# DrorT/demucs

Hardware: AMD Instinct MI355X
Metric: real-time factor (audio-sec/wall-sec) htdemucs 4-stem 44.1kHz stereo, 1/8 GPU (higher is better)
Workload: dtype f32

## Files before the change

### demucs_amd/csrc/gemm_x6.hip

```cpp
#include "gemm_tile.h"
#include "split_bf16.h"

namespace mi {

typedef __attribute__((address_space(1))) const void gvoid_t;
typedef __attribute__((address_space(3))) void lvoid_t;

__global__ void pack_split_kernel(const float *__restrict__ wt, int Kpad, int Mpad, int BM, __bf16 *__restrict__ wx) {
    const size_t idx = blockIdx.x * (size_t)blockDim.x + threadIdx.x;
    if (idx >= (size_t)Kpad * Mpad) return;
    const int k = (int)(idx / Mpad), m = (int)(idx % Mpad);
    const int mt = m / BM, mi = m % BM, kt = k / BK, h = (k % BK) / 8, j = k % 8, nk = Kpad / BK;
    const float x = wt[idx];
    const __bf16 a = (__bf16)x;
    const float r = x - (float)a;
    const __bf16 b = (__bf16)r;
    const __bf16 c = (__bf16)(r - (float)b);
    __bf16 *img = wx + ((size_t)mt * nk + kt) * ((size_t)BM * 48);
    img[((0 * 2 + h) * BM + mi) * 8 + j] = a;
    img[((1 * 2 + h) * BM + mi) * 8 + j] = b;
    img[((2 * 2 + h) * BM + mi) * 8 + j] = c;
}

int launch_pack_split(const float *wt, int Kpad, int Mpad, int tile_m, void *wx, hipStream_t st) {
    MI_REQUIRE(Kpad % BK == 0 && Mpad % tile_m == 0, "pack_split: Kpad %d / Mpad %d do not fit tile %d", Kpad, Mpad, tile_m);
    const size_t n = (size_t)Kpad * Mpad;
    hipLaunchKernelGGL(pack_split_kernel, dim3((unsigned)((n + 255) / 256)), dim3(256), 0, st, wt, Kpad, Mpad, tile_m, (__bf16 *)wx);
    MI_CHECK_LAUNCH();
    return MI_OK;
}

#ifndef MI_X6_ABL
#define MI_X6_ABL 0
#endif
constexpr int kRowTaps = -1;
template <int WM, int WN, int TM, int TN, int EPI, int LFLAGS, bool PLAIN, bool HALF_IMG, int NT>
__device__ __forceinline__ void conv_x6_body(const mi_conv_desc &d, const int N, const int MT, const int Gm) {
    constexpr int BM = WM * TM * 32;
    constexpr bool RAW = PLAIN || NT != 0;
    constexpr bool ROWS = NT == kRowTaps;
    static_assert(NT <= 0 || (!PLAIN && EPI == MI_EPI_GLU), "tap loader: GLU rewrite convs");
    static_assert(!ROWS || (!PLAIN && (EPI == MI_EPI_LINEAR || EPI == MI_EPI_CONVTR || EPI == MI_EPI_GLU)),
                  "row-tap loader: encoder / transposed convs, 1 x 1 + GLU rewrites");
    static_assert(NT >= kRowTaps, "NT: taps, 0 or kRowTaps");
    static_assert(WN * TN * 32 == BN, "block N tile is 128");
    static_assert(WM * WN == 4, "4 waves");
    constexpr int A_BYTES = BM * 96, B_BYTES = BN * 96, STAGE = A_BYTES + B_BYTES;
    constexpr int A_CHUNKS = A_BYTES / 1024;
    static_assert(!HALF_IMG || BM == 64, "HALF_IMG: 64-row tile of a 128-row image");
    constexpr int A_KSTEP = HALF_IMG ? 2 * A_BYTES : A_BYTES, A_CHUNK_STRIDE = HALF_IMG ? 2048 : 1024;
    __shared__ __attribute__((aligned(16))) unsigned char smem[2 * STAGE];
    __shared__ __attribute__((aligned(16))) float braw[RAW ? 2 * BK * BN : 4];

    {
        float agpr_anchor = 0.f;
        asm volatile("; accumulators in AGPRs %0" : "+a"(agpr_anchor));
    }
    const int tid = threadIdx.x, lane = tid & 63;
    const int wave = __builtin_amdgcn_readfirstlane(tid >> 6);
    const int wm = wave / WN, wn = wave % WN;
    int mt, nt;
    if (!tile_of_block(MT, Gm, N, mt, nt)) return;
    const int m0 = mt * BM, n0 = nt * BN;
    const int P = d.O1 * d.O2;
    const int o2v = d.o2_valid ? d.o2_valid : d.O2;
    const int nk = d.Kpad / BK;

    const unsigned char *aimg = reinterpret_cast<const unsigned char *>(d.wx) + (size_t)(HALF_IMG ? mt >> 1 : mt) * nk * A_KSTEP +
                                (HALF_IMG ? (mt & 1) * 1024 : 0) + lane * 16;
#define MI_A_DMA(kt, stage)                                                                                         \
    do {                                                                                                            \
        _Pragma("unroll") for (int c = 0; c < (A_CHUNKS + 3) / 4; ++c) {                                             \
            const int chunk = c * 4 + wave;                                                                         \
            if (chunk < A_CHUNKS)                                                                                   \
                __builtin_amdgcn_global_load_lds((gvoid_t *)(aimg + (size_t)(kt) * A_KSTEP + chunk * A_CHUNK_STRIDE), \
                                                 (lvoid_t *)(smem + (stage) * STAGE + chunk * 1024), 16, 0, 0);     \
        }                                                                                                           \
    } while (0)

    const int bn = tid & 127;
    const int bh = __builtin_amdgcn_readfirstlane(tid >> 7);
    const ColInfo lc = decompose(n0 + bn, N, P, d.O2, PLAIN ? d.O2 : o2v);
    const int i1b = lc.o1 * d.S1, i2b = lc.o2 * d.S2;
    const float *xcol = d.x + (size_t)lc.b * d.x_bstride + (PLAIN ? (size_t)lc.p : (size_t)i1b * (d.x_ld ? d.x_ld : d.D2) + i2b);
    const float *bp = lc.valid ? xcol + (size_t)(8 * bh) * P : d.sink + 256;
    const size_t b_row = lc.valid ? (size_t)P : 0, b_step = lc.valid ? (size_t)BK * P : 0;
    float breg[8];
    const int li = lane & 31, lh = lane >> 5;
    const int rc4 = li * 4, rrow = 4 * wave + lh;
    const ColInfo rcol = decompose(n0 + rc4, N, P, d.O2, NT ? o2v : d.O2);
    const int x_ld = d.x_ld ? d.x_ld : d.D2;
    const int ri1 = rcol.o1 * d.S1;
    const float *rsrc = !rcol.valid ? d.sink + 256
                        : d.x + (size_t)rcol.b * d.x_bstride +
                              (ROWS ? (size_t)ri1 * x_ld + rcol.o2 : (size_t)rcol.p + (NT ? 0 : (size_t)rrow * P));
    const size_t r_row2 = rcol.valid ? (size_t)2 * P : 0, r_step = rcol.valid ? (size_t)BK * P : 0;
    const int4 *ktab4 = reinterpret_cast<const int4 *>(d.ktab) + 4 * wave;
    typedef int v2i __attribute__((ext_vector_type(2)));
    v2i e0, e1, e2, e3;
#define MI_ROW_LOADS "s_load_dwordx2 %0, %4, 0x0\n\ts_load_dwordx2 %1, %4, 0x10\n\ts_load_dwordx2 %2, %4, 0x20\n\t" \
                     "s_load_dwordx2 %3, %4, 0x30\n\t"
#define MI_ROW_ENTRIES(kt)                                                                                          \
    asm volatile(MI_ROW_LOADS "s_waitcnt lgkmcnt(0)"                                                               \
                 : "=&s"(e0), "=&s"(e1), "=&s"(e2), "=&s"(e3) : "s"(ktab4 + (kt) * BK) : "memory")
    constexpr int K2 = 3;
    const int fix_l = (NT && rcol.valid && rcol.o2 == 0) ? 0 : -1;
    const int fr = d.D2 - 1 - rcol.o2;
    const int fix_r = (NT && rcol.valid && fr >= 0 && fr < 4) ? fr : -1;
#define MI_BRAW_DMA(kt, rs)                                                                                         \
    do {                                                                                                            \
        float *dst = braw + (rs) * (BK * BN) + (4 * wave) * BN;                                                     \
        if constexpr (ROWS) {                                                                                       \
            _Pragma("unroll") for (int i = 0; i < 2; ++i) {                                                         \
                const int off = i ? (lh ? e3.x : e2.x) : (lh ? e1.x : e0.x);                                        \
                const int dd1 = i ? (lh ? e3.y : e2.y) : (lh ? e1.y : e0.y);                                        \
                const bool ok = rcol.valid && (unsigned)(ri1 + dd1) < (unsigned)d.D1;                               \
                __builtin_amdgcn_global_load_lds((gvoid_t *)(ok ? rsrc + off : d.sink + 256), (lvoid_t *)(dst + 2 * i * BN), 16, 0, 0); \
            }                                                                                                       \
        } else if constexpr (NT > 0) {                                                                              \
            _Pragma("unroll") for (int i = 0; i < 2; ++i) {                                                         \
                const int k = (kt) * BK + rrow + 2 * i, ci = k / NT, tap = k - ci * NT, t1 = tap / K2, t2 = tap - t1 * K2; \
                const int i1 = rcol.o1 + t1 - d.tap_pad1;                                                           \
                const bool ok = rcol.valid && k < d.K && (unsigned)i1 < (unsigned)d.D1;                             \
                const float *g = rsrc + (int64_t)ci * P + (int64_t)(t1 - d.tap_pad1) * x_ld + (t2 - d.tap_pad2);    \
                __builtin_amdgcn_global_load_lds((gvoid_t *)(ok ? g : d.sink + 256), (lvoid_t *)(dst + 2 * i * BN), 16, 0, 0); \
            }                                                                                                       \
        } else {                                                                                                    \
            const float *g = rsrc + (size_t)(kt) * r_step;                                                          \
            __builtin_amdgcn_global_load_lds((gvoid_t *)g, (lvoid_t *)dst, 16, 0, 0);                               \
            __builtin_amdgcn_global_load_lds((gvoid_t *)(g + r_row2), (lvoid_t *)(dst + 2 * BN), 16, 0, 0);         \
        }                                                                                                           \
    } while (0)
#define MI_BRAW_FIX(kt, rs)                                                                                         \
    do {                                                                                                            \
        if constexpr (NT > 0) {                                                                                     \
            float *row = braw + (rs) * (BK * BN) + rrow * BN + rc4;                                                 \
            _Pragma("unroll") for (int i = 0; i < 2; ++i) {                                                         \
                const int k = (kt) * BK + rrow + 2 * i, dd2 = (k % NT) % K2 - d.tap_pad2;                           \
                if (dd2 < 0 && fix_l >= 0) row[2 * i * BN + fix_l] = 0.f;                                           \
                if (dd2 > 0 && fix_r >= 0) row[2 * i * BN + fix_r] = 0.f;                                           \
            }                                                                                                       \
        }                                                                                                           \
    } while (0)
#define MI_BRAW_READ(rs)                                                                                            \
    do {                                                                                                            \
        _Pragma("unroll") for (int j = 0; j < 8; ++j) breg[j] = braw[(rs) * (BK * BN) + (8 * bh + j) * BN + bn];     \
    } while (0)

#define MI_B_LOAD(kt)                                                                                               \
    do {                                                                                                            \
        if (PLAIN) {                                                                                                \
            _Pragma("unroll") for (int j = 0; j < 8; ++j) breg[j] = bp[(size_t)(kt) * b_step + j * b_row];           \
        } else {                                                                                                    \
            mi_ktab_entry ke[8];                                                                                    \
            _Pragma("unroll") for (int j = 0; j < 8; ++j) ke[j] = d.ktab[(kt) * BK + 8 * bh + j];                    \
            _Pragma("unroll") for (int j = 0; j < 8; ++j) {                                                          \
                bool ok;                                                                                            \
                const float v = gather_b(d, ke[j], xcol, i1b, i2b, lc.valid, ok);                                   \
                breg[j] = ok ? v : 0.f;                                                                             \
            }                                                                                                       \
        }                                                                                                           \
    } while (0)

#define MI_B_STORE(stage)                                                                                           \
    do {                                                                                                            \
        unsigned ph[4], pm[4], pl[4];                                                                               \
        _Pragma("unroll") for (int j = 0; j < 4; ++j) split3(breg[2 * j], breg[2 * j + 1], ph[j], pm[j], pl[j]);    \
        unsigned char *bs = smem + (stage) * STAGE + A_BYTES + (bh * BN + bn) * 16;                                 \
        *reinterpret_cast<uint4 *>(bs) = make_uint4(ph[0], ph[1], ph[2], ph[3]);                                    \
        *reinterpret_cast<uint4 *>(bs + 2 * BN * 16) = make_uint4(pm[0], pm[1], pm[2], pm[3]);                      \
        *reinterpret_cast<uint4 *>(bs + 4 * BN * 16) = make_uint4(pl[0], pl[1], pl[2], pl[3]);                      \
    } while (0)

    f32x16 acc[TM][TN];
#pragma unroll
    for (int a = 0; a < TM; ++a)
#pragma unroll
        for (int b = 0; b < TN; ++b)
#pragma unroll
            for (int r = 0; r < 16; ++r) acc[a][b][r] = 0.f;

    constexpr int PA[6] = {2, 0, 1, 1, 0, 0}, PB[6] = {0, 2, 1, 0, 1, 0};
    MI_A_DMA(0, 0);
    if constexpr (RAW) {
        if constexpr (ROWS) MI_ROW_ENTRIES(0);
        MI_BRAW_DMA(0, 0);
        if (nk > 1) {
            if constexpr (ROWS) MI_ROW_ENTRIES(1);
            MI_BRAW_DMA(1, 1);
        }
        if constexpr (ROWS) { if (nk > 2) MI_ROW_ENTRIES(2); }
        asm volatile("s_waitcnt vmcnt(0)" ::: "memory");
        MI_BRAW_FIX(0, 0);
        if (nk > 1) MI_BRAW_FIX(1, 1);
        __syncthreads();
        MI_BRAW_READ(0);
    } else {
        MI_B_LOAD(0);
    }
    MI_B_STORE(0);
    asm volatile("s_waitcnt vmcnt(0)" ::: "memory");
    __syncthreads();
    int cur = 0;
    bf16x8 keepa[TM][3], keepb[TN][3];
    for (int kt = 0; kt < nk; ++kt) {
        const unsigned char *As = smem + cur * STAGE, *Bs = As + A_BYTES;
        bf16x8 af[TM][3], bf[TN][3];
        if ((MI_X6_ABL & 128) && kt > 0) {
#pragma unroll
            for (int p = 0; p < 3; ++p) {
#pragma unroll
                for (int a = 0; a < TM; ++a) af[a][p] = keepa[a][p];
#pragma unroll
                for (int b = 0; b < TN; ++b) bf[b][p] = keepb[b][p];
            }
        } else
#pragma unroll
        for (int p = 0; p < 3; ++p) {
#pragma unroll
            for (int a = 0; a < TM; ++a)
                af[a][p] = *reinterpret_cast<const bf16x8 *>(As + (((p * 2 + lh) * BM) + (wm * TM + a) * 32 + li) * 16);
#pragma unroll
            for (int b = 0; b < TN; ++b)
                bf[b][p] = *reinterpret_cast<const bf16x8 *>(Bs + (((p * 2 + lh) * BN) + (wn * TN + b) * 32 + li) * 16);
        }
        if (MI_X6_ABL & 128) {
#pragma unroll
            for (int p = 0; p < 3; ++p) {
#pragma unroll
                for (int a = 0; a < TM; ++a) keepa[a][p] = af[a][p];
#pragma unroll
                for (int b = 0; b < TN; ++b) keepb[b][p] = bf[b][p];
            }
        }
        if (MI_X6_ABL & 64) {
            typedef unsigned u32x4 __attribute__((ext_vector_type(4)));
#pragma unroll
            for (int p = 0; p < 3; ++p) {
#pragma unroll
                for (int a = 0; a < TM; ++a) { u32x4 z = __builtin_bit_cast(u32x4, af[a][p]); asm volatile("" : "+v"(z)); af[a][p] = __builtin_bit_cast(bf16x8, z); }
#pragma unroll
                for (int b = 0; b < TN; ++b) { u32x4 z = __builtin_bit_cast(u32x4, bf[b][p]); asm volatile("" : "+v"(z)); bf[b][p] = __builtin_bit_cast(bf16x8, z); }
            }
        }
        if (MI_X6_ABL & 8) {
            typedef unsigned u32x4 __attribute__((ext_vector_type(4)));
#pragma unroll
            for (int p = 0; p < 3; ++p) {
#pragma unroll
                for (int a = 0; a < TM; ++a) { u32x4 z = {0u, 0u, 0u, 0u}; asm volatile("" : "+v"(z)); af[a][p] = __builtin_bit_cast(bf16x8, z); }
#pragma unroll
                for (int b = 0; b < TN; ++b) { u32x4 z = {0u, 0u, 0u, 0u}; asm volatile("" : "+v"(z)); bf[b][p] = __builtin_bit_cast(bf16x8, z); }
            }
        }
        __builtin_amdgcn_sched_barrier(0);
        if (kt + 1 < nk) {
            MI_A_DMA(kt + 1, cur ^ 1);
            if constexpr (RAW) {
                if (kt + 2 < nk) MI_BRAW_DMA(kt + 2, kt & 1);
            } else {
                MI_B_LOAD(kt + 1);
            }
        }
        if constexpr (RAW) {
            MI_BRAW_READ((kt + 1) & 1);
        }
        __builtin_amdgcn_sched_barrier(0);
#pragma unroll
        for (int q = 0; q < 6; ++q)
#pragma unroll
            for (int a = 0; a < TM; ++a)
#pragma unroll
                for (int b = 0; b < TN; ++b)
                    if (!(MI_X6_ABL & 1) || (q == 0 && a == 0 && b == 0)) {
                        acc[a][b] = __builtin_amdgcn_mfma_f32_32x32x16_bf16(af[a][PA[q]], bf[b][PB[q]], acc[a][b], 0, 0, 0);
                        if (MI_X6_ABL & 16) asm volatile("s_nop 15\n\ts_nop 15");
                        if ((MI_X6_ABL & 32) && a == TM - 1 && b == TN - 1) asm volatile("s_nop 15\n\ts_nop 15\n\ts_nop 15\n\ts_nop 15");
                    }
        if (RAW || kt + 1 < nk) MI_B_STORE(cur ^ 1);
        if constexpr (RAW) {
#pragma unroll
            for (int i = 0; i < 6 * TM * TN; ++i) {
                __builtin_amdgcn_sched_group_barrier(0x008, 1, 0);
                __builtin_amdgcn_sched_group_barrier(0x002, (72 + 6 * TM * TN - 1) / (6 * TM * TN), 0);
            }
        }
        if (ROWS && kt + 3 < nk)
            asm volatile(MI_ROW_LOADS "s_waitcnt vmcnt(0) lgkmcnt(0)"
                         : "=&s"(e0), "=&s"(e1), "=&s"(e2), "=&s"(e3) : "s"(ktab4 + (kt + 3) * BK) : "memory");
        else
            asm volatile("s_waitcnt vmcnt(0)" ::: "memory");
        if (kt + 2 < nk) MI_BRAW_FIX(kt + 2, kt & 1);
        __syncthreads();
        cur ^= 1;
    }
#undef MI_A_DMA
#undef MI_B_LOAD
#undef MI_BRAW_DMA
#undef MI_BRAW_FIX
#undef MI_BRAW_READ
#undef MI_ROW_ENTRIES
#undef MI_ROW_LOADS
#undef MI_B_STORE

    if (MI_X6_ABL & 4) {
        float s = 0.f;
        for (int a = 0; a < TM; ++a) for (int b = 0; b < TN; ++b) for (int r = 0; r < 16; ++r) s += acc[a][b][r];
        d.sink[threadIdx.x] = s;
        return;
    }
    conv_epilogue<TM, TN, EPI, LFLAGS>(d, acc, m0, n0, wm, wn, N, P, o2v);
}

template <int WM, int WN, int TM, int TN, int EPI, int LFLAGS, bool PLAIN, bool HALF_IMG = false>
__global__ __launch_bounds__(256, 2) void conv_gemm_x6_kernel(const mi_conv_desc d, const int N, const int MT, const int Gm) {
    conv_x6_body<WM, WN, TM, TN, EPI, LFLAGS, PLAIN, HALF_IMG, 0>(d, N, MT, Gm);
}

template <int WM, int WN, int TM, int TN, bool HALF_IMG, int NT>
__global__ __launch_bounds__(256, 2) void conv_tap_x6_kernel(const mi_conv_desc d, const int N, const int MT, const int Gm) {
    conv_x6_body<WM, WN, TM, TN, MI_EPI_GLU, 0, false, HALF_IMG, NT>(d, N, MT, Gm);
}

template <int WM, int WN, int TM, int TN, int EPI, int LFLAGS, bool HALF_IMG>
__global__ __launch_bounds__(256, 2) void conv_rows_x6_kernel(const mi_conv_desc d, const int N, const int MT, const int Gm) {
    conv_x6_body<WM, WN, TM, TN, EPI, LFLAGS, false, HALF_IMG, kRowTaps>(d, N, MT, Gm);
}

template <int WM, int WN, int TM, int TN, int EPI, int LFLAGS, bool PLAIN, bool HALF_IMG = false, int NTAPS = 0>
static int launch_cfg_x6(const mi_conv_desc &d, hipStream_t st) {
    constexpr int BM = WM * TM * 32;
    const int64_t N64 = (int64_t)d.B * d.O1 * d.O2;
    MI_REQUIRE(N64 < (1ll << 31) - 256, "conv: too many output positions (%lld)", (long long)N64);
    MI_REQUIRE(d.Mpad % (HALF_IMG ? 2 * BM : BM) == 0, "conv: Mpad %d not a multiple of the %d-row tile", d.Mpad, BM);
    const int N = (int)N64, MT = d.Mpad / BM, NT = ceil_div(N, BN);
    const int Gm = pick_m_groups(MT, (size_t)d.Kpad * d.Mpad * 6);
    const unsigned grid = grouped_grid(MT, NT, Gm);
    if constexpr (NTAPS > 0) hipLaunchKernelGGL((conv_tap_x6_kernel<WM, WN, TM, TN, HALF_IMG, NTAPS>), dim3(grid), dim3(256), 0, st, d, N, MT, Gm);
    else if constexpr (NTAPS == kRowTaps)
        hipLaunchKernelGGL((conv_rows_x6_kernel<WM, WN, TM, TN, EPI, LFLAGS, HALF_IMG>), dim3(grid), dim3(256), 0, st, d, N, MT, Gm);
    else hipLaunchKernelGGL((conv_gemm_x6_kernel<WM, WN, TM, TN, EPI, LFLAGS, PLAIN, HALF_IMG>), dim3(grid), dim3(256), 0, st, d, N, MT, Gm);
    MI_CHECK_LAUNCH();
    return MI_OK;
}

template <int EPI, int LFLAGS, bool PLAIN>
static int launch_tile_x6(const mi_conv_desc &d, int tile, hipStream_t st) {
    if constexpr (PLAIN && EPI == MI_EPI_LINEAR) {
        static const int small = getenv("MI_SMALL_TILE") ? atoi(getenv("MI_SMALL_TILE")) : 1;
        if (small && tile == 128 && (int64_t)(d.Mpad / 128) * ceil_div((int64_t)d.B * d.O1 * d.O2, BN) < 200)
            return launch_cfg_x6<1, 4, 2, 1, EPI, LFLAGS, PLAIN, true>(d, st);
    }
    switch (tile) {
        case 128: return launch_cfg_x6<2, 2, 2, 2, EPI, LFLAGS, PLAIN>(d, st);
        case 96: return launch_cfg_x6<1, 4, 3, 1, EPI, LFLAGS, PLAIN>(d, st);
        case 64: return launch_cfg_x6<1, 4, 2, 1, EPI, LFLAGS, PLAIN>(d, st);
    }
    return set_error(MI_EINVAL, "conv x6: unsupported tile_m %d", tile);
}

bool conv_x6_supported(int tile) { return tile == 128 || tile == 96 || tile == 64; }

template <int NT>
static int launch_tile_tap_x6(const mi_conv_desc &d, int tile, hipStream_t st) {
    static const int small = getenv("MI_SMALL_TILE") ? atoi(getenv("MI_SMALL_TILE")) : 1;
    if (small && tile == 128 && (int64_t)(d.Mpad / 128) * ceil_div((int64_t)d.B * d.O1 * d.O2, BN) < 200)
        return launch_cfg_x6<1, 4, 2, 1, MI_EPI_GLU, 0, false, true, NT>(d, st);
    if (tile == 128) return launch_cfg_x6<2, 2, 2, 2, MI_EPI_GLU, 0, false, false, NT>(d, st);
    return launch_cfg_x6<1, 4, 3, 1, MI_EPI_GLU, 0, false, false, NT>(d, st);
}

int launch_conv_tap_x6(const mi_conv_desc &d, int tile, hipStream_t st) {
    g_last_conv_route = 7;
    MI_REQUIRE(d.wx && ((uintptr_t)d.wx & 15) == 0, "conv tap x6: split weight image missing or misaligned");
    MI_REQUIRE(d.epi == MI_EPI_GLU && (tile == 96 || tile == 128) && (d.ntaps == 9 || d.ntaps == 3),
               "conv tap x6: GLU layer with 9 or 3 taps on a 96- or 128-row tile (epi %d, tile %d, ntaps %d)", d.epi, tile, d.ntaps);
    return d.ntaps == 9 ? launch_tile_tap_x6<9>(d, tile, st) : launch_tile_tap_x6<3>(d, tile, st);
}

template <int EPI, int LFLAGS>
static int launch_tile_rows_x6(const mi_conv_desc &d, int tile, hipStream_t st) {
    static const int small = getenv("MI_SMALL_TILE") ? atoi(getenv("MI_SMALL_TILE")) : 1;
    if (small && tile == 128 && (int64_t)(d.Mpad / 128) * ceil_div((int64_t)d.B * d.O1 * d.O2, BN) < 200)
        return launch_cfg_x6<1, 4, 2, 1, EPI, LFLAGS, false, true, kRowTaps>(d, st);
    if (tile == 128) return launch_cfg_x6<2, 2, 2, 2, EPI, LFLAGS, false, false, kRowTaps>(d, st);
    return launch_cfg_x6<1, 4, 3, 1, EPI, LFLAGS, false, false, kRowTaps>(d, st);
}

int launch_conv_rows_x6(const mi_conv_desc &d, int tile, hipStream_t st) {
    g_last_conv_route = 8;
    MI_REQUIRE(d.wx && ((uintptr_t)d.wx & 15) == 0, "conv rows x6: split weight image missing or misaligned");
    MI_REQUIRE(d.ktab && ((uintptr_t)d.ktab & 63) == 0, "conv rows x6: gather table missing or misaligned");
    MI_REQUIRE(tile == 96 || tile == 128, "conv rows x6: 96- or 128-row tile (tile %d)", tile);
    if (d.epi == MI_EPI_CONVTR) return launch_tile_rows_x6<MI_EPI_CONVTR, 0>(d, tile, st);
    if (d.epi == MI_EPI_GLU) {
        MI_REQUIRE(tile == 128, "conv rows x6: GLU on a 128-row tile (tile %d)", tile);
        return launch_tile_rows_x6<MI_EPI_GLU, 0>(d, tile, st);
    }
    MI_REQUIRE(d.epi == MI_EPI_LINEAR && (d.flags & (MI_FLAG_GELU | MI_FLAG_SCALE | MI_FLAG_RES | MI_FLAG_LN | MI_FLAG_STATS)) == MI_FLAG_GELU,
               "conv rows x6: LINEAR + GELU, CONVTR or GLU (epi %d, flags %d)", d.epi, d.flags);
    return launch_tile_rows_x6<MI_EPI_LINEAR, MI_FLAG_GELU>(d, tile, st);
}

int launch_conv_x6(const mi_conv_desc &d, int tile, bool plain, hipStream_t st) {
    g_last_conv_route = 4;
    MI_REQUIRE(d.wx && ((uintptr_t)d.wx & 15) == 0, "conv x6: split weight image missing or misaligned");
#define MI_DISPATCH(E)                                              \
    case E: return plain ? launch_tile_x6<E, 0, true>(d, tile, st) : launch_tile_x6<E, 0, false>(d, tile, st)
#define MI_LINEAR(F)                                                \
    case F: return plain ? launch_tile_x6<MI_EPI_LINEAR, F, true>(d, tile, st) : launch_tile_x6<MI_EPI_LINEAR, F, false>(d, tile, st)
    if (d.epi == MI_EPI_LINEAR) {
        switch (d.flags & (MI_FLAG_GELU | MI_FLAG_SCALE | MI_FLAG_RES | MI_FLAG_LN | MI_FLAG_STATS)) {
            MI_LINEAR(0);
            MI_LINEAR(MI_FLAG_GELU);
            MI_LINEAR(MI_FLAG_RES);
            MI_LINEAR(MI_FLAG_SCALE | MI_FLAG_RES);
            MI_LINEAR(MI_FLAG_SCALE | MI_FLAG_RES | MI_FLAG_STATS);
            MI_LINEAR(MI_FLAG_LN);
            MI_LINEAR(MI_FLAG_LN | MI_FLAG_GELU);
        }
        return set_error(MI_EINVAL, "conv: unsupported LINEAR flag combination %d", d.flags);
    }
#undef MI_LINEAR
    switch (d.epi) {
        MI_DISPATCH(MI_EPI_GLU);
        MI_DISPATCH(MI_EPI_BIAS_STATS);
        MI_DISPATCH(MI_EPI_STATS_ONLY);
        MI_DISPATCH(MI_EPI_GN_GLU);
        MI_DISPATCH(MI_EPI_CONVTR);
    }
#undef MI_DISPATCH
    return set_error(MI_EINVAL, "conv: unsupported epilogue %d", d.epi);
}

}
```

Baseline: 2315.

## Deepen conv GEMM LDS pipeline to three-stage rings with partial vmcnt waits

Moves the x6 conv GEMM shared memory to a dynamically sized buffer, with a three-stage ring for the A weight tiles and the raw B tiles when they fit in an 80 KB budget. DMA for A and B is issued further ahead, and the full vmcnt(0) drain is replaced by counted partial waits, so loads for later K steps can stay in flight across the barrier. It also adds an opt-in timestamp probe behind a compile flag. The cost is more LDS per workgroup, which needs an attribute raise above 48 KB and may limit occupancy, plus more complex counter bookkeeping that is easy to get wrong.

```diff
diff --git a/demucs_amd/csrc/gemm_x6.hip b/demucs_amd/csrc/gemm_x6.hip
--- a/demucs_amd/csrc/gemm_x6.hip
+++ b/demucs_amd/csrc/gemm_x6.hip
@@ -1,10 +1,9 @@
 #include "gemm_tile.h"
 #include "split_bf16.h"
+#include <vector>
+#include <atomic>
 
 namespace mi {
-
-typedef __attribute__((address_space(1))) const void gvoid_t;
-typedef __attribute__((address_space(3))) void lvoid_t;
 
 __global__ void pack_split_kernel(const float *__restrict__ wt, int Kpad, int Mpad, int BM, __bf16 *__restrict__ wx) {
     const size_t idx = blockIdx.x * (size_t)blockDim.x + threadIdx.x;
@@ -34,6 +33,62 @@
 #define MI_X6_ABL 0
 #endif
 constexpr int kRowTaps = -1;
+
+#ifndef MI_X6_STAMP
+#define MI_X6_STAMP 0
+#endif
+#if MI_X6_STAMP
+constexpr int kStampWaves = 4 * 4096, kStampVals = 10;
+__device__ unsigned long long g_x6_stamps[kStampWaves * kStampVals];
+#define MI_STAMP_NOW(t)                                                                                             \
+    do {                                                                                                            \
+        __builtin_amdgcn_sched_barrier(0);                                                                          \
+        asm volatile("s_memtime %0\n\ts_waitcnt lgkmcnt(0)" : "=s"(t)::"memory");                                   \
+        __builtin_amdgcn_sched_barrier(0);                                                                          \
+    } while (0)
+#define MI_STAMP_BEGIN()                                                                                            \
+    unsigned long long st_sum[7] = {0, 0, 0, 0, 0, 0, 0}, st_prev, st_now, st_t0, st_r0;                            \
+    asm volatile("s_memrealtime %0\n\ts_waitcnt lgkmcnt(0)" : "=s"(st_r0)::"memory");                              \
+    MI_STAMP_NOW(st_prev);                                                                                          \
+    st_t0 = st_prev
+#define MI_STAMP_SEG(i)                                                                                             \
+    do {                                                                                                            \
+        MI_STAMP_NOW(st_now);                                                                                       \
+        st_sum[i] += st_now - st_prev;                                                                              \
+        st_prev = st_now;                                                                                           \
+    } while (0)
+#define MI_STAMP_END()                                                                                              \
+    do {                                                                                                            \
+        unsigned long long st_r1;                                                                                   \
+        asm volatile("s_memrealtime %0\n\ts_waitcnt lgkmcnt(0)" : "=s"(st_r1)::"memory");                          \
+        const unsigned w = blockIdx.x * 4 + wave;                                                                   \
+        if (lane == 0 && w < (unsigned)kStampWaves) {                                                               \
+            unsigned long long *o = g_x6_stamps + (size_t)w * kStampVals;                                           \
+            for (int i = 0; i < 7; ++i) o[i] = st_sum[i];                                                           \
+            o[7] = (unsigned long long)nk;                                                                          \
+            o[8] = st_prev - st_t0;                                                                                 \
+            o[9] = st_r1 - st_r0;                                                                                   \
+        }                                                                                                           \
+    } while (0)
+#else
+#define MI_STAMP_BEGIN() do {} while (0)
+#define MI_STAMP_SEG(i) do {} while (0)
+#define MI_STAMP_END() do {} while (0)
+#endif
+
+#ifndef MI_X6_A3
+#define MI_X6_A3 0
+#endif
+template <int BM, bool RAW>
+struct x6_lds {
+    static constexpr int A_BYTES = BM * 96, B_BYTES = BN * 96, R_BYTES = BK * BN * 4, BUDGET = 80 * 1024;
+    static constexpr bool FITS = 3 * A_BYTES + 2 * B_BYTES + (RAW ? 3 * R_BYTES : 0) <= BUDGET;
+    static constexpr int A_ST = (FITS || MI_X6_A3) ? 3 : 2;
+    static constexpr int R_ST = !RAW ? 0 : (FITS || !MI_X6_A3) ? 3 : 2;
+    static constexpr int B_OFF = A_ST * A_BYTES, R_OFF = B_OFF + 2 * B_BYTES, BYTES = R_OFF + R_ST * R_BYTES;
+    static_assert(BYTES <= BUDGET && A_BYTES % 16 == 0, "two workgroups per CU");
+};
+
 template <int WM, int WN, int TM, int TN, int EPI, int LFLAGS, bool PLAIN, bool HALF_IMG, int NT>
 __device__ __forceinline__ void conv_x6_body(const mi_conv_desc &d, const int N, const int MT, const int Gm) {
     constexpr int BM = WM * TM * 32;
@@ -45,12 +100,15 @@
     static_assert(NT >= kRowTaps, "NT: taps, 0 or kRowTaps");
     static_assert(WN * TN * 32 == BN, "block N tile is 128");
     static_assert(WM * WN == 4, "4 waves");
-    constexpr int A_BYTES = BM * 96, B_BYTES = BN * 96, STAGE = A_BYTES + B_BYTES;
+    constexpr int A_BYTES = BM * 96, B_BYTES = BN * 96;
     constexpr int A_CHUNKS = A_BYTES / 1024;
     static_assert(!HALF_IMG || BM == 64, "HALF_IMG: 64-row tile of a 128-row image");
     constexpr int A_KSTEP = HALF_IMG ? 2 * A_BYTES : A_BYTES, A_CHUNK_STRIDE = HALF_IMG ? 2048 : 1024;
-    __shared__ __attribute__((aligned(16))) unsigned char smem[2 * STAGE];
-    __shared__ __attribute__((aligned(16))) float braw[RAW ? 2 * BK * BN : 4];
+    using L = x6_lds<BM, RAW>;
+    constexpr int A_ST = L::A_ST, R_ST = L::R_ST;
+    extern __shared__ __attribute__((aligned(16))) unsigned char x6_smem[];
+    unsigned char *const smem = x6_smem, *const bsm = x6_smem + L::B_OFF;
+    float *const braw = reinterpret_cast<float *>(x6_smem + L::R_OFF);
 
     {
         float agpr_anchor = 0.f;
@@ -68,13 +126,13 @@
 
     const unsigned char *aimg = reinterpret_cast<const unsigned char *>(d.wx) + (size_t)(HALF_IMG ? mt >> 1 : mt) * nk * A_KSTEP +
                                 (HALF_IMG ? (mt & 1) * 1024 : 0) + lane * 16;
+    const int na = (A_CHUNKS - wave + 3) / 4;
 #define MI_A_DMA(kt, stage)                                                                                         \
     do {                                                                                                            \
         _Pragma("unroll") for (int c = 0; c < (A_CHUNKS + 3) / 4; ++c) {                                             \
             const int chunk = c * 4 + wave;                                                                         \
-            if (chunk < A_CHUNKS)                                                                                   \
-                __builtin_amdgcn_global_load_lds((gvoid_t *)(aimg + (size_t)(kt) * A_KSTEP + chunk * A_CHUNK_STRIDE), \
-                                                 (lvoid_t *)(smem + (stage) * STAGE + chunk * 1024), 16, 0, 0);     \
+            if (A_CHUNKS % 4 == 0 || chunk < A_CHUNKS)                                                              \
+                lds_dma16(aimg + (size_t)(kt) * A_KSTEP + chunk * A_CHUNK_STRIDE, smem + (stage) * A_BYTES + chunk * 1024); \
         }                                                                                                           \
     } while (0)
 
@@ -115,7 +173,7 @@
                 const int off = i ? (lh ? e3.x : e2.x) : (lh ? e1.x : e0.x);                                        \
                 const int dd1 = i ? (lh ? e3.y : e2.y) : (lh ? e1.y : e0.y);                                        \
                 const bool ok = rcol.valid && (unsigned)(ri1 + dd1) < (unsigned)d.D1;                               \
-                __builtin_amdgcn_global_load_lds((gvoid_t *)(ok ? rsrc + off : d.sink + 256), (lvoid_t *)(dst + 2 * i * BN), 16, 0, 0); \
+                lds_dma16(ok ? rsrc + off : d.sink + 256, dst + 2 * i * BN); \
             }                                                                                                       \
         } else if constexpr (NT > 0) {                                                                              \
             _Pragma("unroll") for (int i = 0; i < 2; ++i) {                                                         \
@@ -123,12 +181,12 @@
                 const int i1 = rcol.o1 + t1 - d.tap_pad1;                                                           \
                 const bool ok = rcol.valid && k < d.K && (unsigned)i1 < (unsigned)d.D1;                             \
                 const float *g = rsrc + (int64_t)ci * P + (int64_t)(t1 - d.tap_pad1) * x_ld + (t2 - d.tap_pad2);    \
-                __builtin_amdgcn_global_load_lds((gvoid_t *)(ok ? g : d.sink + 256), (lvoid_t *)(dst + 2 * i * BN), 16, 0, 0); \
+                lds_dma16(ok ? g : d.sink + 256, dst + 2 * i * BN); \
             }                                                                                                       \
         } else {                                                                                                    \
             const float *g = rsrc + (size_t)(kt) * r_step;                                                          \
-            __builtin_amdgcn_global_load_lds((gvoid_t *)g, (lvoid_t *)dst, 16, 0, 0);                               \
-            __builtin_amdgcn_global_load_lds((gvoid_t *)(g + r_row2), (lvoid_t *)(dst + 2 * BN), 16, 0, 0);         \
+            lds_dma16(g, dst);                          \
+            lds_dma16(g + r_row2, dst + 2 * BN);         \
         }                                                                                                           \
     } while (0)
 #define MI_BRAW_FIX(kt, rs)                                                                                         \
@@ -166,7 +224,7 @@
     do {                                                                                                            \
         unsigned ph[4], pm[4], pl[4];                                                                               \
         _Pragma("unroll") for (int j = 0; j < 4; ++j) split3(breg[2 * j], breg[2 * j + 1], ph[j], pm[j], pl[j]);    \
-        unsigned char *bs = smem + (stage) * STAGE + A_BYTES + (bh * BN + bn) * 16;                                 \
+        unsigned char *bs = bsm + (stage) * B_BYTES + (bh * BN + bn) * 16;                                 \
         *reinterpret_cast<uint4 *>(bs) = make_uint4(ph[0], ph[1], ph[2], ph[3]);                                    \
         *reinterpret_cast<uint4 *>(bs + 2 * BN * 16) = make_uint4(pm[0], pm[1], pm[2], pm[3]);                      \
         *reinterpret_cast<uint4 *>(bs + 4 * BN * 16) = make_uint4(pl[0], pl[1], pl[2], pl[3]);                      \
@@ -181,30 +239,68 @@
             for (int r = 0; r < 16; ++r) acc[a][b][r] = 0.f;
 
     constexpr int PA[6] = {2, 0, 1, 1, 0, 0}, PB[6] = {0, 2, 1, 0, 1, 0};
-    MI_A_DMA(0, 0);
+
+#define MI_VM_CASE(N) case N: asm volatile("s_waitcnt vmcnt(" #N ")" ::: "memory"); break;
+#define MI_WAIT_VM(n)                                                                                               \
+    switch (n) {                                                                                                    \
+        MI_VM_CASE(1) MI_VM_CASE(2) MI_VM_CASE(3) MI_VM_CASE(4) MI_VM_CASE(5)                                       \
+        default: asm volatile("s_waitcnt vmcnt(0)" ::: "memory");            \
+    }
+#define MI_ROWS_CASE(N, t) case N: asm volatile(MI_ROW_LOADS "s_waitcnt vmcnt(" #N ") lgkmcnt(0)"                  \
+                                               : "=&s"(e0), "=&s"(e1), "=&s"(e2), "=&s"(e3) : "s"(ktab4 + (t) * BK) : "memory"); break;
+#define MI_WAIT_VM_ROWS(n, t)                                                                                       \
+    switch (n) {                                                                                                    \
+        MI_ROWS_CASE(1, t) MI_ROWS_CASE(2, t) MI_ROWS_CASE(3, t) MI_ROWS_CASE(4, t) MI_ROWS_CASE(5, t)              \
+        default: asm volatile(MI_ROW_LOADS "s_waitcnt vmcnt(0) lgkmcnt(0)"                                          \
+                              : "=&s"(e0), "=&s"(e1), "=&s"(e2), "=&s"(e3) : "s"(ktab4 + (t) * BK) : "memory");     \
+    }
+#define MI_BARRIER() asm volatile("s_waitcnt lgkmcnt(0)\n\ts_barrier" ::: "memory")
+    static_assert(A_ST == 2 || A_ST == 3, "A ring: two or three stages");
+    static_assert(!RAW || R_ST == 2 || R_ST == 3, "raw ring: two or three slots");
+    {
+        int n = 0;
+        MI_A_DMA(0, 0);
+        if constexpr (RAW) {
+            if constexpr (ROWS) MI_ROW_ENTRIES(0);
+            MI_BRAW_DMA(0, 0);
+            if (nk > 1) {
+                if constexpr (ROWS) MI_ROW_ENTRIES(1);
+                MI_BRAW_DMA(1, 1);
+            }
+        }
+        if constexpr (A_ST == 3) {
+            if (nk > 1) { MI_A_DMA(1, 1); n += na; }
+        }
+        if constexpr (RAW && R_ST == 3) {
+            if (nk > 2) {
+                if constexpr (ROWS) MI_ROW_ENTRIES(2);
+                MI_BRAW_DMA(2, 2);
+                n += 2;
+            }
+        }
+        if constexpr (ROWS) { if (nk > R_ST) MI_ROW_ENTRIES(R_ST); }
+        MI_WAIT_VM(n);
+    }
     if constexpr (RAW) {
-        if constexpr (ROWS) MI_ROW_ENTRIES(0);
-        MI_BRAW_DMA(0, 0);
-        if (nk > 1) {
-            if constexpr (ROWS) MI_ROW_ENTRIES(1);
-            MI_BRAW_DMA(1, 1);
-        }
-        if constexpr (ROWS) { if (nk > 2) MI_ROW_ENTRIES(2); }
-        asm volatile("s_waitcnt vmcnt(0)" ::: "memory");
         MI_BRAW_FIX(0, 0);
         if (nk > 1) MI_BRAW_FIX(1, 1);
-        __syncthreads();
+        MI_BARRIER();
         MI_BRAW_READ(0);
     } else {
         MI_B_LOAD(0);
     }
     MI_B_STORE(0);
-    asm volatile("s_waitcnt vmcnt(0)" ::: "memory");
-    __syncthreads();
+    MI_BARRIER();
     int cur = 0;
+    int as = 0, rs = 0;
     bf16x8 keepa[TM][3], keepb[TN][3];
+    MI_STAMP_BEGIN();
     for (int kt = 0; kt < nk; ++kt) {
-        const unsigned char *As = smem + cur * STAGE, *Bs = As + A_BYTES;
+        MI_STAMP_SEG(6);
+        const int as_prev = as == 0 ? A_ST - 1 : as - 1;
+        const int rs_next = RAW ? (rs + 1 == R_ST ? 0 : rs + 1) : 0;
+        const int rs_fix = R_ST == 3 ? (rs == 0 ? 2 : rs - 1) : rs;
+        const unsigned char *As = smem + as * A_BYTES, *Bs = bsm + cur * B_BYTES;
         bf16x8 af[TM][3], bf[TN][3];
         if ((MI_X6_ABL & 128) && kt > 0) {
 #pragma unroll
@@ -253,18 +349,23 @@
                 for (int b = 0; b < TN; ++b) { u32x4 z = {0u, 0u, 0u, 0u}; asm volatile("" : "+v"(z)); bf[b][p] = __builtin_bit_cast(bf16x8, z); }
             }
         }
+        MI_STAMP_SEG(0);
         __builtin_amdgcn_sched_barrier(0);
-        if (kt + 1 < nk) {
-            MI_A_DMA(kt + 1, cur ^ 1);
-            if constexpr (RAW) {
-                if (kt + 2 < nk) MI_BRAW_DMA(kt + 2, kt & 1);
-            } else {
-                MI_B_LOAD(kt + 1);
-            }
-        }
+        int n = 0;
+        if constexpr (A_ST == 2) { if (kt + 1 < nk) MI_A_DMA(kt + 1, as_prev); }
+        if constexpr (RAW && R_ST == 2) { if (kt + 2 < nk) MI_BRAW_DMA(kt + 2, rs); }
+        if constexpr (A_ST == 3) {
+            if (kt + 2 < nk) { MI_A_DMA(kt + 2, as_prev); n += na; }
+        }
+        if constexpr (RAW && R_ST == 3) {
+            if (kt + 3 < nk) { MI_BRAW_DMA(kt + 3, rs); n += 2; }
+        }
+        if constexpr (!RAW) { if (kt + 1 < nk) MI_B_LOAD(kt + 1); }
+        MI_STAMP_SEG(1);
         if constexpr (RAW) {
-            MI_BRAW_READ((kt + 1) & 1);
-        }
+            MI_BRAW_READ(rs_next);
+        }
+        MI_STAMP_SEG(2);
         __builtin_amdgcn_sched_barrier(0);
 #pragma unroll
         for (int q = 0; q < 6; ++q)
@@ -285,15 +386,26 @@
                 __builtin_amdgcn_sched_group_barrier(0x002, (72 + 6 * TM * TN - 1) / (6 * TM * TN), 0);
             }
         }
-        if (ROWS && kt + 3 < nk)
-            asm volatile(MI_ROW_LOADS "s_waitcnt vmcnt(0) lgkmcnt(0)"
-                         : "=&s"(e0), "=&s"(e1), "=&s"(e2), "=&s"(e3) : "s"(ktab4 + (kt + 3) * BK) : "memory");
-        else
-            asm volatile("s_waitcnt vmcnt(0)" ::: "memory");
-        if (kt + 2 < nk) MI_BRAW_FIX(kt + 2, kt & 1);
-        __syncthreads();
+        MI_STAMP_SEG(3);
+        if (ROWS && kt + 1 + R_ST < nk) {
+            MI_WAIT_VM_ROWS(n, kt + 1 + R_ST);
+        } else {
+            MI_WAIT_VM(n);
+        }
+        MI_STAMP_SEG(4);
+        if (kt + 2 < nk) MI_BRAW_FIX(kt + 2, rs_fix);
+        MI_BARRIER();
+        MI_STAMP_SEG(5);
         cur ^= 1;
-    }
+        as = as + 1 == A_ST ? 0 : as + 1;
+        rs = rs_next;
+    }
+    MI_STAMP_END();
+#undef MI_VM_CASE
+#undef MI_WAIT_VM
+#undef MI_ROWS_CASE
+#undef MI_WAIT_VM_ROWS
+#undef MI_BARRIER
 #undef MI_A_DMA
 #undef MI_B_LOAD
 #undef MI_BRAW_DMA
@@ -325,6 +437,24 @@
 template <int WM, int WN, int TM, int TN, int EPI, int LFLAGS, bool HALF_IMG>
 __global__ __launch_bounds__(256, 2) void conv_rows_x6_kernel(const mi_conv_desc d, const int N, const int MT, const int Gm) {
     conv_x6_body<WM, WN, TM, TN, EPI, LFLAGS, false, HALF_IMG, kRowTaps>(d, N, MT, Gm);
+}
+
+template <auto KERNEL, int LDS>
+static int launch_ring_x6(unsigned grid, hipStream_t st, const mi_conv_desc &d, int N, int MT, int Gm) {
+    static_assert(LDS % 16 == 0 && LDS <= 80 * 1024, "two workgroups per CU");
+    if (LDS > 48 * 1024) {
+        static std::atomic<unsigned long long> raised{0};
+        int dev = 0;
+        MI_REQUIRE(hipGetDevice(&dev) == hipSuccess && dev >= 0 && dev < 64, "conv x6: device %d", dev);
+        if (!(raised.load(std::memory_order_acquire) >> dev & 1ull)) {
+            MI_REQUIRE(hipFuncSetAttribute((const void *)KERNEL, hipFuncAttributeMaxDynamicSharedMemorySize, LDS) == hipSuccess,
+                       "conv x6: %d bytes of dynamic LDS refused", LDS);
+            raised.fetch_or(1ull << dev, std::memory_order_release);
+        }
+    }
+    hipLaunchKernelGGL(KERNEL, dim3(grid), dim3(256), LDS, st, d, N, MT, Gm);
+    MI_CHECK_LAUNCH();
+    return MI_OK;
 }
 
 template <int WM, int WN, int TM, int TN, int EPI, int LFLAGS, bool PLAIN, bool HALF_IMG = false, int NTAPS = 0>
@@ -336,12 +466,11 @@
     const int N = (int)N64, MT = d.Mpad / BM, NT = ceil_div(N, BN);
     const int Gm = pick_m_groups(MT, (size_t)d.Kpad * d.Mpad * 6);
     const unsigned grid = grouped_grid(MT, NT, Gm);
-    if constexpr (NTAPS > 0) hipLaunchKernelGGL((conv_tap_x6_kernel<WM, WN, TM, TN, HALF_IMG, NTAPS>), dim3(grid), dim3(256), 0, st, d, N, MT, Gm);
+    constexpr int LDS = x6_lds<BM, PLAIN || NTAPS != 0>::BYTES;
+    if constexpr (NTAPS > 0) return launch_ring_x6<conv_tap_x6_kernel<WM, WN, TM, TN, HALF_IMG, NTAPS>, LDS>(grid, st, d, N, MT, Gm);
     else if constexpr (NTAPS == kRowTaps)
-        hipLaunchKernelGGL((conv_rows_x6_kernel<WM, WN, TM, TN, EPI, LFLAGS, HALF_IMG>), dim3(grid), dim3(256), 0, st, d, N, MT, Gm);
-    else hipLaunchKernelGGL((conv_gemm_x6_kernel<WM, WN, TM, TN, EPI, LFLAGS, PLAIN, HALF_IMG>), dim3(grid), dim3(256), 0, st, d, N, MT, Gm);
-    MI_CHECK_LAUNCH();
-    return MI_OK;
+        return launch_ring_x6<conv_rows_x6_kernel<WM, WN, TM, TN, EPI, LFLAGS, HALF_IMG>, LDS>(grid, st, d, N, MT, Gm);
+    else return launch_ring_x6<conv_gemm_x6_kernel<WM, WN, TM, TN, EPI, LFLAGS, PLAIN, HALF_IMG>, LDS>(grid, st, d, N, MT, Gm);
 }
 
 template <int EPI, int LFLAGS, bool PLAIN>
@@ -434,3 +563,13 @@
 }
 
 }
+
+#if MI_X6_STAMP
+extern "C" int mi_debug_x6_stamps(void *dst, size_t bytes) {
+    if (!dst) {
+        const std::vector<unsigned long long> zero((size_t)mi::kStampWaves * mi::kStampVals);
+        return hipMemcpyToSymbol(HIP_SYMBOL(mi::g_x6_stamps), zero.data(), zero.size() * sizeof(unsigned long long)) == hipSuccess ? 0 : 1;
+    }
+    return hipMemcpyFromSymbol(dst, HIP_SYMBOL(mi::g_x6_stamps), bytes) == hipSuccess ? 0 : 1;
+}
+#endif
```

New measurement: 2285. -1.3%, worse.
